# StanfordASL/GuSTO.jl

Measured on AMD Instinct MI355X. Metric: converged trajectories/sec (batched SCP), freeflyer_se2 N=50, inputs resident in HBM, higher is better.
Workload: dtype f64

## Files before the change

gusto.jl_amd/csrc/common.hpp:

```cpp
#pragma once
#include <hip/hip_runtime.h>
#include <math.h>
#include <stdint.h>

#include "gusto_hip.h"

namespace gusto {

#define GD __device__ __forceinline__
typedef double v4d __attribute__((ext_vector_type(4)));

constexpr int ROW_HARD = 0;
constexpr int ROW_PEN = 1;
constexpr int ROW_PEN_TR = 2;
constexpr int ROW_PEN_EQ = 3;
constexpr int ROW_HARD_EQ = 4;
constexpr int ROW_EQ = 5;
GD bool row_is_hard(int kind) { return kind == ROW_HARD || kind == ROW_HARD_EQ; }

constexpr int RS_T = 0, RS_LAM = 1, RS_LAMB = 2, RS_S = 3, RS_DT = 4, RS_DL = 5, RS_DS = 6, RS_KA = 7, RS_KB = 8,
              RS_NVAR = 9;

#ifndef GUSTO_DUBINS_WAVES
#define GUSTO_DUBINS_WAVES 2
#endif
#ifndef GUSTO_WAVES_PER_EU
#define GUSTO_WAVES_PER_EU 1
#endif

#ifndef GUSTO_TO_SWEEP_CALL
#define GUSTO_TO_SWEEP_CALL true
#endif
#ifndef GUSTO_TO4_SWEEP_CALL
#define GUSTO_TO4_SWEEP_CALL true
#endif
#ifndef GUSTO_USE_MFMA
#define GUSTO_USE_MFMA true
#endif
constexpr int GUSTO_TO_FREEFLYER_SE2 = 4, GUSTO_TO_ASTROBEE_SE3 = 5, GUSTO_TO_ASTROBEE_SE3_MANIFOLD = 6;
constexpr double TRAJOPT_DEFECT_REG = 1e-4;
constexpr int RS_EARLIER = 0, RS_ROW = 1, RS_ROW_LANE = 2;
template <int MODEL> struct MT;
template <> struct MT<GUSTO_FREEFLYER_SE2> {
    static constexpr int NDEF = 0;
    static constexpr int n = 6, m = 3, WS = 2, NFIX = 3, NHU = 2;
    static constexpr int WAVES_PER_EU = GUSTO_WAVES_PER_EU;
    static constexpr int RS_FORM = RS_ROW;
    static constexpr bool SWEEP_CALL = false;
    static constexpr bool MFMA = false;
    static constexpr int SCHED_PROBE = 2;
    static constexpr int SCHED_SLICE = 4;
    static constexpr bool LTI = true, HAS_OBS = true;
    static constexpr bool PG2 = true;
    static constexpr int pg_r0(int c) { return c < 3 ? c : (c < 6 ? c - 3 : c - 6); }
    static constexpr int pg_r1(int c) { return c < 3 ? c + 3 : (c < 6 ? c : c - 3); }
    static constexpr bool Anz(int i, int j) { return j == i + 3; }
    static constexpr bool Mnz(int i, int j) { return i == j || j == i + 3; }
    static constexpr bool Bnz(int i, int j) { return i == j + 3; }
    static constexpr bool Gnz(int i, int j) { return i == j || i == j + 3; }
    static constexpr bool Hnz(int, int) { return true; }
};
template <> struct MT<GUSTO_DUBINS_CAR> {
    static constexpr int NDEF = 0;
    static constexpr int n = 3, m = 1, WS = 2, NFIX = 6, NHU = 2;
    static constexpr int WAVES_PER_EU = GUSTO_DUBINS_WAVES;
    static constexpr int RS_FORM = RS_ROW;
    static constexpr bool SWEEP_CALL = false;
    static constexpr bool MFMA = false;
    static constexpr int SCHED_PROBE = 1; static constexpr int SCHED_SLICE = 0;
    static constexpr bool LTI = false, HAS_OBS = false;
    static constexpr bool PG2 = false;
    static constexpr int pg_r0(int) { return 0; }
    static constexpr int pg_r1(int) { return 0; }
    static constexpr bool Anz(int, int) { return true; }
    static constexpr bool Mnz(int, int) { return true; }
    static constexpr bool Bnz(int, int) { return true; }
    static constexpr bool Gnz(int, int) { return true; }
    static constexpr bool Hnz(int, int) { return true; }
};
template <> struct MT<GUSTO_ASTROBEE_SE3> {
    static constexpr int NDEF = 0;
    static constexpr int n = 12, m = 6, WS = 3, NFIX = 3, NHU = 2;
    static constexpr int WAVES_PER_EU = 1;
    static constexpr int RS_FORM = RS_ROW_LANE;
    static constexpr bool SWEEP_CALL = true;
    static constexpr bool MFMA = GUSTO_USE_MFMA;
    static constexpr int SCHED_PROBE = 1; static constexpr int SCHED_SLICE = 0;
    static constexpr bool LTI = false, HAS_OBS = true;
    static constexpr bool PG2 = false;
    static constexpr int pg_r0(int) { return 0; }
    static constexpr int pg_r1(int) { return 0; }
    static constexpr bool Anz(int i, int j) { return i < 3 ? j == i + 3 : (i < 6 ? false : (i < 9 ? j >= 6 : j >= 9)); }
    static constexpr bool Mnz(int i, int j) { return i < 3 ? (j == i || j == i + 3) : (i < 6 ? j == i : (i < 9 ? j >= 6 : j >= 9)); }
    static constexpr bool Bnz(int i, int j) { return j < 3 ? i == j + 3 : i == j + 6; }
    static constexpr bool Gnz(int i, int j) { return j < 3 ? (i == j || i == j + 3) : i >= 6; }
    static constexpr bool Hnz(int i, int j) { return i / 3 == j / 3; }
};
template <> struct MT<GUSTO_ASTROBEE_SE3_MANIFOLD> {
    static constexpr int NDEF = 0;
    static constexpr int n = 13, m = 6, WS = 3, NFIX = 5, NHU = 2;
    static constexpr int WAVES_PER_EU = 1;
    static constexpr int RS_FORM = RS_EARLIER;
    static constexpr bool SWEEP_CALL = true ;
    static constexpr bool MFMA = GUSTO_USE_MFMA;
    static constexpr int SCHED_PROBE = 1; static constexpr int SCHED_SLICE = 0;
    static constexpr bool LTI = false, HAS_OBS = true;
    static constexpr bool PG2 = false;
    static constexpr int pg_r0(int) { return 0; }
    static constexpr int pg_r1(int) { return 0; }
    static constexpr bool Anz(int i, int j) { return i < 3 ? j == i + 3 : (i < 6 ? false : (i < 10 ? j >= 6 : j >= 10)); }
    static constexpr bool Mnz(int i, int j) { return i < 3 ? (j == i || j == i + 3) : (i < 6 ? j == i : (i < 10 ? j >= 6 : j >= 10)); }
    static constexpr bool Bnz(int i, int j) { return j < 3 ? i == j + 3 : i == j + 7; }
    static constexpr bool Gnz(int i, int j) { return j < 3 ? (i == j || i == j + 3) : i >= 6; }
    static constexpr int hblk(int i) { return i < 3 ? 0 : (i < 6 ? 1 : (i < 10 ? 2 : 3)); }
    static constexpr bool Hnz(int i, int j) { return hblk(i) == hblk(j); }
};

template <> struct MT<GUSTO_TO_FREEFLYER_SE2> {
    using G = MT<GUSTO_FREEFLYER_SE2>;
    static constexpr int NDEF = 6, n = 6, m = 3 + NDEF, WS = 2, NFIX = 3, NHU = 2 + 2 * NDEF;
    static constexpr int WAVES_PER_EU = 1, SCHED_PROBE = 0, SCHED_SLICE = 0;
    static constexpr int RS_FORM = RS_ROW;
    static constexpr bool SWEEP_CALL = GUSTO_TO4_SWEEP_CALL, MFMA = false, LTI = false, HAS_OBS = true, PG2 = false;
    static constexpr int pg_r0(int) { return 0; }
    static constexpr int pg_r1(int) { return 0; }
    static constexpr bool Anz(int i, int j) { return G::Anz(i, j); }
    static constexpr bool Mnz(int i, int j) { return G::Mnz(i, j); }
    static constexpr bool Bnz(int i, int j) { return j < G::m && G::Bnz(i, j); }
    static constexpr bool Gnz(int i, int j) { return j < G::m ? G::Gnz(i, j) : i == j - G::m; }
    static constexpr bool Hnz(int, int) { return true; }
};
template <> struct MT<GUSTO_TO_ASTROBEE_SE3> {
    using G = MT<GUSTO_ASTROBEE_SE3>;
    static constexpr int NDEF = 12, n = 12, m = 6 + NDEF, WS = 3, NFIX = 3, NHU = 2 + 2 * NDEF;
    static constexpr int WAVES_PER_EU = 1, SCHED_PROBE = 0, SCHED_SLICE = 0;
    static constexpr int RS_FORM = RS_ROW;
    static constexpr bool SWEEP_CALL = GUSTO_TO_SWEEP_CALL, MFMA = false, LTI = false, HAS_OBS = true, PG2 = false;
    static constexpr int pg_r0(int) { return 0; }
    static constexpr int pg_r1(int) { return 0; }
    static constexpr bool Anz(int i, int j) { return G::Anz(i, j); }
    static constexpr bool Mnz(int i, int j) { return G::Mnz(i, j); }
    static constexpr bool Bnz(int i, int j) { return j < G::m && G::Bnz(i, j); }
    static constexpr bool Gnz(int i, int j) { return j < G::m ? G::Gnz(i, j) : i == j - G::m; }
    static constexpr bool Hnz(int, int) { return true; }
};

template <> struct MT<GUSTO_TO_ASTROBEE_SE3_MANIFOLD> {
    using G = MT<GUSTO_ASTROBEE_SE3_MANIFOLD>;
    static constexpr int NDEF = 13, n = 13, m = 6 + NDEF, WS = 3, NFIX = 5, NHU = 2 + 2 * NDEF;
    static constexpr int WAVES_PER_EU = 1, SCHED_PROBE = 0, SCHED_SLICE = 0;
    static constexpr int RS_FORM = RS_ROW;
    static constexpr bool SWEEP_CALL = GUSTO_TO_SWEEP_CALL, MFMA = false, LTI = false, HAS_OBS = true, PG2 = false;
    static constexpr int pg_r0(int) { return 0; }
    static constexpr int pg_r1(int) { return 0; }
    static constexpr bool Anz(int i, int j) { return G::Anz(i, j); }
    static constexpr bool Mnz(int i, int j) { return G::Mnz(i, j); }
    static constexpr bool Bnz(int i, int j) { return j < G::m && G::Bnz(i, j); }
    static constexpr bool Gnz(int i, int j) { return j < G::m ? G::Gnz(i, j) : i == j - G::m; }
    static constexpr bool Hnz(int, int) { return true; }
};
constexpr double TRAJOPT_EQ_DELTA = 1e-8;

inline void warm_defaults(int model, gusto_ipm_opts& io) {
    if (io.mu_floor < 0) io.mu_floor = (model == GUSTO_ASTROBEE_SE3_MANIFOLD) ? 1e-10 : 1e-11;
    if (io.sigma_max < 0) io.sigma_max = (model == GUSTO_TO_FREEFLYER_SE2 || model == GUSTO_TO_ASTROBEE_SE3 || model == GUSTO_TO_ASTROBEE_SE3_MANIFOLD) ? 0.0 : 0.1;
    if (!(io.mu_warm < 0)) { if (io.mu_warm_gain < 0) io.mu_warm_gain = 0.0; return; }
    switch (model) {
    case GUSTO_DUBINS_CAR: io.mu_warm = 1e-9; io.mu_warm_gain = 0.0; io.mu_warm_max = 1e-9; break;
    case GUSTO_FREEFLYER_SE2: io.mu_warm = 1e-4; io.mu_warm_gain = 0.1; io.mu_warm_max = 1e-2; break;
    case GUSTO_ASTROBEE_SE3: io.mu_warm = 1e-6; io.mu_warm_gain = 1.0; io.mu_warm_max = 1e-2; break;
    default: io.mu_warm = 1e-4; io.mu_warm_gain = 1.0; io.mu_warm_max = 1e-2; break;
    }
}
constexpr double IPM_DIVERGED = 1e3;
GD double warm_mu(const gusto_ipm_opts& io, double c) {
    if (io.mu_warm == 0.0) return 0.0;
    return fmin(fmax(io.mu_warm, io.mu_warm_max), fmax(io.mu_warm, io.mu_warm_gain * c * c));
}

GD constexpr int sidx(int i, int j, int n) {
    return i <= j ? i * n - i * (i - 1) / 2 + (j - i) : j * n - j * (j - 1) / 2 + (i - j);
}

template <int MODEL> struct Rec {
    using T = MT<MODEL>;
    static constexpr int n = T::n, m = T::m, NZ = n + m;
    static constexpr int r64(int c) { return (c + 63) / 64 * 64; }
    static constexpr bool S_TRI = false;
    static constexpr int NS = S_TRI ? m * (m + 1) / 2 : m * m;
    static constexpr int SQQ = r64(NZ * (NZ + 1) / 2), SNN = r64(n * n + 1), SKD = r64(2 * m * n + NS + 1);
    static constexpr int oK = 0, oD = m * n, oS = 2 * m * n;
    static constexpr int KD_DUMMY = 2 * m * n + NS;
    static constexpr int sS(int i, int l) {
        if (!S_TRI) return oS + i * m + l;
        const int a = i < l ? i : l, b = i < l ? l : i;
        return oS + a * m - a * (a - 1) / 2 + (b - a);
    }
};

template <int MODEL> struct SpPG {
    using T = MT<MODEL>;
    static constexpr int n = T::n, m = T::m;
    static constexpr int pos_phi(int l, int i) {
        int c = 0;
        for (int i2 = 0; i2 < n; i2++)
            for (int l2 = 0; l2 < n; l2++)
                if (T::Mnz(l2, i2) && (i2 < i || (i2 == i && l2 < l))) c++;
        return c;
    }
    static constexpr int NPHI = pos_phi(0, n);
    static constexpr int pos_gam(int l, int j) {
        int c = NPHI;
        for (int l2 = 0; l2 < n; l2++)
            for (int j2 = 0; j2 < m; j2++)
                if (T::Gnz(l2, j2) && (l2 < l || (l2 == l && j2 < j))) c++;
        return c;
    }
    static constexpr int NS = pos_gam(n, 0);
    static constexpr int S = (NS + 15) / 16 * 16;
    static constexpr bool USE = T::MFMA && T::NDEF == 0;
};

template <int MODEL> constexpr int rs_stride_rt(int N) { return MT<MODEL>::RS_FORM == RS_EARLIER ? N : (N + 63) & ~63; }
template <int MODEL, bool ONE> GD int rs_stride(int N) {
    if constexpr (ONE && MT<MODEL>::RS_FORM != RS_EARLIER) return 64;
    else return rs_stride_rt<MODEL>(N);
}
template <int MODEL, bool ONE> constexpr int rs_form() { return (ONE && MT<MODEL>::RS_FORM == RS_ROW_LANE) ? RS_ROW : MT<MODEL>::RS_FORM; }

struct WsLayout {
    int nslot;
    size_t rowstate, obs_nh, obs_c0, obs_mask, PG, PGS, QQ, Paft, Piaft, KD, Phicl, pvt, to_traj, total;
};
template <int MODEL> inline WsLayout make_ws_layout(int N, int n_obs) {
    using T = MT<MODEL>;
    constexpr int n = T::n, m = T::m, NZ = n + m;
    WsLayout L;
    L.nslot = T::NFIX + n_obs + 2 * n + T::NHU;
    size_t o = 0;
    auto take = [&](size_t c) { size_t r = o; o += (c + 1) & ~size_t(1); return r; };
    L.rowstate = take((size_t)RS_NVAR * L.nslot * rs_stride_rt<MODEL>(N));
    L.obs_nh = take((size_t)n_obs * T::WS * N);
    L.obs_c0 = take((size_t)n_obs * N);
    L.obs_mask = take((size_t)N);
    L.PG = take((size_t)(T::LTI ? 1 : N) * n * NZ);
    L.PGS = take(SpPG<MODEL>::USE ? (size_t)N * SpPG<MODEL>::S : 0);
    using R = Rec<MODEL>;
    L.QQ = take((size_t)N * R::SQQ);
    L.Paft = take((size_t)(N + 1) * R::SNN) + R::SNN;
    L.Piaft = take((size_t)(N + 1) * R::SNN) + R::SNN;
    L.KD = take((size_t)N * R::SKD);
    L.Phicl = take((size_t)N * R::SNN);
    L.pvt = take((size_t)N * (5 * n + 5 * m));
    L.to_traj = take(T::NDEF > 0 ? (size_t)2 * N * (n + m) : 0);
    L.total = T::RS_FORM == RS_EARLIER ? o : (o + 15) & ~size_t(15);
    return L;
}

template <int MODEL, bool ONE> struct LdsC {
    using T = MT<MODEL>;
    static constexpr int n = T::n, m = T::m, NZ = n + m;
    static constexpr bool BIG = n > 8;
    static constexpr int NPGB = (ONE && !T::LTI) ? 2 : 3;
    static constexpr int sP = 0, sPi = sP + n * n, sPG = sPi + n * n, sT0 = sPG + NPGB * n * NZ,
                         sHh = sT0 + ((ONE && BIG) ? 0 : n * NZ), sZ = sHh + NZ * NZ, sT = (ONE && BIG) ? sZ : sT0,
                         sGd = sZ + NZ * n, misc = sGd + ((ONE && BIG) ? 1 : 2) * n * n, sgoal = misc + 64 , lut = misc + 80,
                         vecs1w = (lut + (NZ * (NZ + 1) / 2 + 1) / 2 + 1 + 1) & ~1,
                         sK = vecs1w, sD = sK + m * n, sW = sD + m * n, sV = sW + m * n, vecsmw = sV + m * n,
                         vecs = ONE ? vecs1w : vecsmw;
    static constexpr int NVN = 7, NVM = 1;
    static constexpr bool KD_LDS = ONE && n <= 8;
    static constexpr bool PHI_FROM_K = KD_LDS && T::PG2;
    static constexpr bool PG_LDS = ONE && !T::LTI && n <= 4;
    static constexpr bool LC_LDS = ONE && MODEL == GUSTO_DUBINS_CAR;
    static constexpr int KDW = 2 * m * n + m * (m + 1) / 2;
    static constexpr int KDS = (KDW > NZ * (NZ + 1) / 2) ? KDW : NZ * (NZ + 1) / 2;
    static constexpr bool PHICL_LDS = n <= 8 && !PHI_FROM_K;
};
#ifndef GUSTO_SEG_W2
#ifdef GUSTO_STRICT_SYNC
#define GUSTO_SEG_W2 0
#else
#define GUSTO_SEG_W2 1
#endif
#endif
#ifndef GUSTO_SEG_MIN_N
#define GUSTO_SEG_MIN_N 4
#endif
template <int MODEL> constexpr bool seg2_big() { return GUSTO_SEG_W2 && MT<MODEL>::MFMA && MT<MODEL>::SWEEP_CALL && MT<MODEL>::NDEF == 0; }
__host__ __device__ constexpr int seg_lo(int c, int N, int NCH) { return (int)((long)N * c / NCH); }
constexpr int SEGW_FACTOR = 1, SEGW_BACK = 2, SEGW_FWD = 3, SEGW_ROWS_R = 5, SEGW_STEP = 6, SEGW_STEP_CS = 7, SEGW_EXIT = 9;
constexpr int SEG_RP = 15;
template <int MODEL, int NCH> struct SegB {
    static constexpr int n = MT<MODEL>::n, m = MT<MODEL>::m, NNp = (n * n + 1) & ~1, NPG = n * (n + m), NI = NCH - 1;
    static constexpr int IFB = 7 * NNp, Tt = 0, Sg = NNp, Pa = 2 * NNp, A2 = 3 * NNp, A3 = 4 * NNp, Pc = 5 * NNp, PIc = 6 * NNp;
    static constexpr int IF(int j) { return j * IFB; }
    static constexpr int CHB = 3 * NNp, Pf = 0, Pif = NNp, Gdf = 2 * NNp;
    static constexpr int CH(int c) { return NI * IFB + c * CHB; }
    static constexpr int COM = NI * (IFB + CHB), Gci = COM, A1 = COM + NNp, X1 = COM + 2 * NNp, X2 = COM + 3 * NNp;
    static constexpr int vec = COM + 4 * NNp;
    static constexpr int XI(int j) { return vec + 16 * j; }
    static constexpr int LAM(int j) { return vec + 16 * NI + 16 * j; }
    static constexpr int PBV(int c) { return vec + 32 * NI + 16 * (c - 1); }
    static constexpr int hlp = vec + 48 * NI, HLB = (2 * NPG + 64 > SEG_RP * 64) ? 2 * NPG + 64 : SEG_RP * 64;
// ... 373 lines not shown
```

gusto.jl_amd/csrc/ipm.hpp:

```cpp
#pragma once
#include "rows.hpp"

#ifndef GUSTO_COOP_CHOL_MIN
#define GUSTO_COOP_CHOL_MIN 7
#endif

namespace gusto {

extern __shared__ __attribute__((aligned(16))) double gusto_dyn_lds[];

template <int MODEL> constexpr bool costate_adjoint();

struct IpmOut {
    int status, iters;
    double obj, res_p, res_d, mu;
};

template <bool ONEWAVE> GD void blk_sync() {
    if constexpr (ONEWAVE) {
#ifdef GUSTO_STRICT_SYNC
        asm volatile("s_waitcnt vmcnt(0) lgkmcnt(0)\n\ts_barrier" ::: "memory");
#endif
        __builtin_amdgcn_fence(__ATOMIC_ACQ_REL, "wavefront");
        __builtin_amdgcn_wave_barrier();
// ... 1088 lines not shown
                    for (int l = 0; l < n; l++) pb[l] = ex[sg * n + l];
#pragma unroll
                    for (int l = 0; l < n; l++) acc[l % PS] += col[l] * pb[l];
                } else {
                    double pb[n];
#pragma unroll
                    for (int l = 0; l < n; l++) pb[l] = readlane_f64(pval, sg * n + l);
                    __builtin_amdgcn_sched_barrier(0);
#pragma unroll
                    for (int l = 0; l < n; l++) acc[l % PS] += col[l] * pb[l];
                }
                const double s = (PS == 4) ? (acc[0] + acc[1]) + (acc[2] + acc[PS - 1]) : acc[0];
                pval = (g == gs) ? s : pval;
                if constexpr (XL) ex[tid] = pval;
            }
        }
        {
            const int kk = k0 - g;
            if (tid < C * n && kk >= 1) K.pv[(kk - 1) * n + i] = pval;
        }
#pragma unroll
        for (int l = 0; l < n; l++) col[l] = coln[l];
        qv = qvn;
    }
    K.sync();
}

template <class BLKA> GD void forward_sweep_1w(BLKA K) {
    using BLK = std::remove_cv_t<std::remove_reference_t<BLKA>>;
    constexpr int n = BLK::n, C = 64 / n, PS = n > 8 ? 4 : 1;
    constexpr bool XL = n > 8;
    double* ex = K.sHh;
    using R = typename BLK::R;
    const int tid = K.tid, N = K.N;
    const int g = (tid < C * n) ? tid / n : C - 1, i = (tid < C * n) ? tid % n : 0;
    double gi = 0.0;
    auto phi_e = [&](int r_, int c_) { return (r_ == c_) ? 1.0 : ((c_ == r_ + n / 2) ? K.dt : 0.0); };
    if constexpr (BLK::C::PHI_FROM_K) {
        constexpr int m = BLK::m;
        double Bd[n * m];
        Dyn<BLK::MODEL_ID>::B(*K.mpp, Bd);
        const double h = 0.5 * K.dt;
#pragma unroll
        for (int l = 0; l < n; l++) {
            const int c_ = l % m;
            const double hb = h * Bd[(c_ + n / 2) * m + c_];
            const double gv = (l < n / 2) ? 2.0 * (h * hb) : 2.0 * hb;
            gi = (i == l) ? gv : gi;
        }
    }
    double phr[n];
#pragma unroll
    for (int l = 0; l < n; l++) phr[l] = phi_e(i, l);
    double row[n], rown[n], cv, cvn = 0, yval = 0.0;
    auto fetch = [&](int k0, double* r, double& c) {
        const int kk = (k0 + g < N) ? k0 + g : N - 1;
        if constexpr (BLK::C::PHI_FROM_K) {
            constexpr int m = BLK::m;
            const int ic = (i < m) ? i : i - m;
#pragma unroll
            for (int l = 0; l < n; l++) r[l] = phr[l] - gi * K.kdl[kk * BLK::C::KDS + ic * n + l];
        } else if constexpr (n <= 4) {
            const bool ok = k0 + g < N;
#pragma unroll
            for (int l = 0; l < n; l++) r[l] = ok ? K.Phicl[(size_t)kk * BLK::SPH + i * n + l] : 0.0;
            c = ok ? K.dY[kk * n + i] : 0.0;
            return;
        } else {
#pragma unroll
            for (int l = 0; l < n; l++) r[l] = K.Phicl[(size_t)kk * BLK::SPH + i * n + l];
        }
        c = K.dY[kk * n + i];
    };
    constexpr int RING = (XL && !BLK::C::KD_LDS) ? GUSTO_SWEEP_RING : 1;
    if constexpr (RING > 1) {
        double rb[RING][n], qb[RING];
#pragma unroll
        for (int d = 0; d < RING - 1; d++) fetch(d * C, rb[d], qb[d]);
        ex[tid] = yval;
        K.sync();
        for (int kb = 0; kb < N; kb += RING * C) {
            static_for<0, RING>([&](auto DD) {
                constexpr int d = decltype(DD)::value;
                const int k0 = kb + d * C;
                fetch(k0 + (RING - 1) * C, rb[(d + RING - 1) % RING], qb[(d + RING - 1) % RING]);
                if (k0 < N) {
#pragma unroll
                    for (int gs = 0; gs < C; gs++) {
                        if (k0 + gs < N) {
                            const int sg = (gs == 0) ? C - 1 : gs - 1;
                            double acc[PS];
#pragma unroll
                            for (int q = 0; q < PS; q++) acc[q] = (q == 0) ? qb[d] : 0.0;
                            double pb[n];
#pragma unroll
                            for (int l = 0; l < n; l++) pb[l] = readlane_f64(yval, sg * n + l);
                            __builtin_amdgcn_sched_barrier(0);
#pragma unroll
                            for (int l = 0; l < n; l++) acc[l % PS] += rb[d][l] * pb[l];
                            const double s = (PS == 4) ? (acc[0] + acc[1]) + (acc[2] + acc[PS - 1]) : acc[0];
                            yval = (g == gs) ? s : yval;
                        }
                    }
                    const int kk = k0 + g;
                    if (tid < C * n && kk < N) K.dY[kk * n + i] = yval;
                }
            });
        }
        K.sync();
        return;
    }
    fetch(0, row, cv);
    if constexpr (XL) ex[tid] = yval;
    K.sync();
    for (int k0 = 0; k0 < N; k0 += C) {
        if (k0 + C < N) fetch(k0 + C, rown, cvn);
#pragma unroll
        for (int gs = 0; gs < C; gs++) {
            if (k0 + gs < N) {
                const int sg = (gs == 0) ? C - 1 : gs - 1;
                double acc[PS];
#pragma unroll
                for (int q = 0; q < PS; q++) acc[q] = (q == 0) ? cv : 0.0;
                if constexpr (XL) {
                    double pb[n];
#pragma unroll
                    for (int l = 0; l < n; l++) pb[l] = ex[sg * n + l];
#pragma unroll
                    for (int l = 0; l < n; l++) acc[l % PS] += row[l] * pb[l];
                } else {
                    double pb[n];
#pragma unroll
                    for (int l = 0; l < n; l++) pb[l] = readlane_f64(yval, sg * n + l);
                    __builtin_amdgcn_sched_barrier(0);
#pragma unroll
                    for (int l = 0; l < n; l++) acc[l % PS] += row[l] * pb[l];
                }
                const double s = (PS == 4) ? (acc[0] + acc[1]) + (acc[2] + acc[PS - 1]) : acc[0];
                yval = (g == gs) ? s : yval;
                if constexpr (XL) ex[tid] = yval;
            }
        }
        {
            const int kk = k0 + g;
            if (tid < C * n && kk < N) K.dY[kk * n + i] = yval;
        }
#pragma unroll
        for (int l = 0; l < n; l++) row[l] = rown[l];
        cv = cvn;
    }
    K.sync();
}

template <int MODEL> GD void costate_pass_1w(SweepView<MODEL> K, const double* mugn) {
    using T = MT<MODEL>;
    using R = Rec<MODEL>;
    constexpr int n = T::n, C = 64 / n;
    const int tid = K.tid, N = K.N;
    const int g = (tid < C * n) ? tid / n : C - 1, i = (tid < C * n) ? tid % n : 0;
    double mg[n];
#pragma unroll
    for (int l = 0; l < n; l++) mg[l] = mugn[l];
    constexpr int RING = GUSTO_SWEEP_RING;
    double pr[RING][n], pi[RING][n];
    auto fetch = [&](int k0, double* a, double* b) {
        const int k = (k0 + g + 1 < N) ? k0 + g : N - 2;
        const double* pa = K.Paft + (size_t)k * R::SNN + (T::MFMA ? i : i * n);
        const double* pb = K.Piaft + (size_t)k * R::SNN + (T::MFMA ? i : i * n);
#pragma unroll
        for (int l = 0; l < n; l++) { a[l] = pa[T::MFMA ? l * n : l]; b[l] = pb[T::MFMA ? l * n : l]; }
    };
#pragma unroll
    for (int d = 0; d < RING - 1; d++) fetch(d * C, pr[d], pi[d]);
    for (int kb = 0; kb + 1 < N; kb += RING * C) {
        static_for<0, RING>([&](auto DD) {
            constexpr int d = decltype(DD)::value;
            const int k0 = kb + d * C;
            fetch(k0 + (RING - 1) * C, pr[(d + RING - 1) % RING], pi[(d + RING - 1) % RING]);
            if (k0 + 1 < N) {
                const bool ok = tid < C * n && k0 + g + 1 < N;
                const int k = (k0 + g + 1 < N) ? k0 + g : N - 2;
                double s = K.pv[k * n + i] - K.rv[k * n + i];
#pragma unroll
                for (int l = 0; l < n; l++) s += pr[d][l] * K.dY[k * n + l] + pi[d][l] * mg[l];
                if (ok) K.nun[(k + 1) * n + i] = s;
            }
        });
    }
    K.sync();
}
template <int MODEL> __device__ __noinline__ void costate_pass_1w_call(typename Blk<MODEL, true>::Args a) {
    Blk<MODEL, true> B(a, gusto_dyn_lds);
    costate_pass_1w<MODEL>(SweepView<MODEL>::make(B), gusto_dyn_lds + LdsC<MODEL, true>::misc + 48);
}


template <int MODEL> constexpr bool adjoint_pattern_ok() {
    using T = MT<MODEL>;
    constexpr int n = T::n, q = n - 9;
    for (int i = 0; i < n; i++)
        for (int l = 0; l < n; l++) {
            const bool want = (i < 6) ? (l == i || (i >= 3 && l == i - 3)) : (l >= 6 && l < ((i < 6 + q) ? 6 + q : n));
            if (want != T::Mnz(l, i)) return false;
        }
    return true;
}
template <int MODEL> GD void adjoint_sweep_1w(SweepView<MODEL> K) {
    using T = MT<MODEL>;
    constexpr int n = T::n, NZ = T::n + T::m, C = 64 / n, q = n - 9, NR = n - 6;
    static_assert(adjoint_pattern_ok<MODEL>(), "column pattern of M of the astrobee models");
    const int tid = K.tid, N = K.N;
    const int g = (tid < C * n) ? tid / n : C - 1, i = (tid < C * n) ? tid % n : 0;
    int rl[NR];
    bool rok[NR];
    const int hi = (i < 6 + q) ? 6 + q : n;
#pragma unroll
    for (int j = 0; j < NR; j++) {
        rl[j] = (i < 6) ? ((j == 1 && i >= 3) ? i - 3 : i) : 6 + j;
        rok[j] = (i < 6) ? (j == 0 || (j == 1 && i >= 3)) : (6 + j < hi);
        if (!rok[j]) rl[j] = i;
    }
    int cs = 0, pj[NR];
#pragma unroll
    for (int i2 = 0; i2 < n; i2++) cs = (i == i2) ? SpPG<MODEL>::pos_phi(0, i2) : cs;
#pragma unroll
    for (int j = 0; j < NR; j++) pj[j] = (i < 6) ? ((i >= 3) ? (j == 1 ? 0 : (j == 0 ? 1 : 0)) : 0) : (rok[j] ? j : 0);
    double* ex = K.sHh;
    constexpr int RING = GUSTO_SWEEP_RING;
    double cb[RING][NR], vb[RING];
    auto fetch = [&](int k0, double* c, double& v) {
        const int kk = (k0 - g >= 1) ? k0 - g : 1;
        const auto pg = K.PGS + (size_t)kk * SpPG<MODEL>::S + cs;
#pragma unroll
        for (int j = 0; j < NR; j++) { const double a = pg[pj[j]]; c[j] = rok[j] ? a : 0.0; }
        v = K.nun[kk * n + i];
    };
#pragma unroll
    for (int d = 0; d < RING - 1; d++) fetch(N - 2 - d * C, cb[d], vb[d]);
    double val = K.nun[(N - 1) * n + i];
    ex[tid] = val;
    K.sync();
    for (int kb = N - 2; kb >= 1; kb -= RING * C) {
        static_for<0, RING>([&](auto DD) {
            constexpr int d = decltype(DD)::value;
            const int k0 = kb - d * C;
            fetch(k0 - (RING - 1) * C, cb[(d + RING - 1) % RING], vb[(d + RING - 1) % RING]);
            if (k0 >= 1) {
#pragma unroll
                for (int gs = 0; gs < C; gs++) {
                    if (k0 - gs >= 1) {
                        const int sg = (gs == 0) ? C - 1 : gs - 1;
                        double pb[NR];
#pragma unroll
                        for (int j = 0; j < NR; j++) pb[j] = ex[sg * n + rl[j]];
                        double s = vb[d];
#pragma unroll
                        for (int j = 0; j < NR; j++) s += cb[d][j] * pb[j];
                        val = (g == gs) ? s : val;
                        ex[tid] = val;
                    }
                }
                const int kk = k0 - g;
                if (tid < C * n && kk >= 1) K.nun[kk * n + i] = val;
            }
        });
    }
    K.sync();
}
template <int MODEL> __device__ __noinline__ void adjoint_sweep_1w_call(typename Blk<MODEL, true>::Args a, double hdt) {
    using T = MT<MODEL>;
    constexpr int n = T::n, m = T::m;
    Blk<MODEL, true> K(a, gusto_dyn_lds);
    adjoint_sweep_1w<MODEL>(SweepView<MODEL>::make(K));
    if (K.tid == 0) {
        const double* gxs = gusto_dyn_lds + LdsC<MODEL, true>::misc + 16;
        double Ad[n * n], x0[n], u0[m];
#pragma unroll
        for (int i = 0; i < n; i++) x0[i] = K.Xp[i];
#pragma unroll
        for (int i = 0; i < m; i++) u0[i] = K.Up[i];
        Dyn<MODEL>::A(K.P.mp, x0, u0, Ad);
#pragma unroll
        for (int i = 0; i < n; i++) {
            double s = gxs[i] + K.nun[n + i];
#pragma unroll
            for (int j = 0; j < n; j++) if (T::Anz(j, i)) s += hdt * Ad[j * n + i] * K.nun[n + j];
            K.nun[i] = -s;
        }
    }
    K.sync();
}

template <int MODEL> __device__ __noinline__ void factor_sweep_1w_call(typename Blk<MODEL, true>::Args a, Prof* pf) {
    Blk<MODEL, true> B(a, gusto_dyn_lds);
    SweepView<MODEL> K = SweepView<MODEL>::make(B);
    if constexpr (MT<MODEL>::MFMA) {
        if constexpr (!costate_adjoint<MODEL>()) factor_sweep_mfma<MODEL, false>(K, gusto_dyn_lds + LdsC<MODEL, true>::misc + 8, *pf);
        else if (costate_adjoint_now<MODEL>()) factor_sweep_mfma<MODEL, true>(K, gusto_dyn_lds + LdsC<MODEL, true>::misc + 8, *pf);
        else factor_sweep_mfma<MODEL, false>(K, gusto_dyn_lds + LdsC<MODEL, true>::misc + 8, *pf);
    }
    else factor_sweep_1w<MODEL>(K, gusto_dyn_lds + LdsC<MODEL, true>::misc + 8, *pf);
}
template <int MODEL, class BLK> __device__ __noinline__ void factor_sweep_mw_call(typename BLK::Args a, Prof* pf) {
    BLK K(a, gusto_dyn_lds);
    if constexpr (MT<MODEL>::m >= GUSTO_COOP_CHOL_MIN) {
        if (K.NTr <= 64) { factor_sweep_w1<MODEL>(K, gusto_dyn_lds + BLK::C::misc + 8, *pf); return; }
    }
    factor_sweep_mw<MODEL>(K, gusto_dyn_lds + BLK::C::misc + 8, *pf);
}
template <class BLK> __device__ __noinline__ void backward_sweep_mw_call(typename BLK::Args a) {
    BLK K(a, gusto_dyn_lds);
    if (K.NTr <= 64) backward_sweep_1w<const BLK&>(K); else backward_sweep_mw(K);
}
template <class BLK> __device__ __noinline__ void forward_sweep_mw_call(typename BLK::Args a) {
    BLK K(a, gusto_dyn_lds);
    if (K.NTr <= 64) forward_sweep_1w<const BLK&>(K); else forward_sweep_mw(K);
}
template <int MODEL, class BLK> GD void factor_sweep(BLK& K, double* fail, Prof& pf) {
    if constexpr (!BLK::ONE && MT<MODEL>::SWEEP_CALL && MT<MODEL>::NDEF > 0) factor_sweep_mw_call<MODEL, BLK>(K.args(), &pf);
    else if constexpr (!BLK::ONE) factor_sweep_mw<MODEL>(K, fail, pf);
    else if constexpr (MT<MODEL>::SWEEP_CALL) factor_sweep_1w_call<MODEL>(K.args(), &pf);
    else if constexpr (MT<MODEL>::MFMA) factor_sweep_mfma<MODEL, false>(SweepView<MODEL>::make(K), fail, pf);
    else if constexpr (MT<MODEL>::PG2 && LdsC<MODEL, true>::KD_LDS) {
        factor_sweep_pg2<MODEL>(SweepView<MODEL>::make(K), fail, pf);
    }
    else factor_sweep_1w<MODEL>(SweepView<MODEL>::make(K), fail, pf);
}
template <int MODEL> __device__ __noinline__ void backward_sweep_1w_call(typename Blk<MODEL, true>::Args a) {
    Blk<MODEL, true> B(a, gusto_dyn_lds);
    backward_sweep_1w(SweepView<MODEL>::make(B));
}
template <int MODEL> __device__ __noinline__ void forward_sweep_1w_call(typename Blk<MODEL, true>::Args a) {
    Blk<MODEL, true> B(a, gusto_dyn_lds);
    forward_sweep_1w(SweepView<MODEL>::make(B));
}
template <int MODEL, class BLK> GD void backward_sweep(BLK& K) {
    if constexpr (!BLK::ONE && MT<MODEL>::SWEEP_CALL && MT<MODEL>::NDEF > 0) backward_sweep_mw_call<BLK>(K.args());
    else if constexpr (!BLK::ONE) backward_sweep_mw(K);
    else if constexpr (MT<MODEL>::SWEEP_CALL) backward_sweep_1w_call<MODEL>(K.args());
    else backward_sweep_1w(SweepView<MODEL>::make(K));
}
template <int MODEL, class BLK> GD void forward_sweep(BLK& K) {
    if constexpr (!BLK::ONE && MT<MODEL>::SWEEP_CALL && MT<MODEL>::NDEF > 0) forward_sweep_mw_call<BLK>(K.args());
    else if constexpr (!BLK::ONE) forward_sweep_mw(K);
    else if constexpr (MT<MODEL>::SWEEP_CALL) forward_sweep_1w_call<MODEL>(K.args());
    else forward_sweep_1w(SweepView<MODEL>::make(K));
}

template <int MODEL, class BLK> GD void inv_spd_block(BLK& K, double* fail) {
    constexpr int n = BLK::n;
    const int tid = K.tid, nt = K.nt();
    double* A = K.sGd;
    double* Li = K.sHh;
    if constexpr (BLK::ONE) {
        const int r = tid < n ? tid : n - 1;
        double a[n];
#pragma unroll
        for (int c = 0; c < n; c++) { a[c] = A[r * n + c]; if (c == r && !K.is_goal(r)) a[c] = 1.0; }
        bool bad = false;
        static_for<0, n>([&](auto J) {
            constexpr int j = decltype(J)::value;
            const double ajj = readlane_f64(a[j], j);
            if (!(ajj > 0.0)) bad = true;
            const double d = rsqrt_nr(ajj);
            a[j] = (r >= j) ? a[j] * d : a[j];
            static_for<j + 1, n>([&](auto C) {
                constexpr int c = decltype(C)::value;
                const double lcj = readlane_f64(a[j], c);
                double t = a[c];
                t -= a[j] * lcj;
                a[c] = (r >= c) ? t : a[c];
            });
        });
        if (bad) *fail = 1.0;
        double x[n];
        static_for<0, n>([&](auto I) {
            constexpr int i = decltype(I)::value;
            const double ri = rcp_nr(readlane_f64(a[i], i));
            double acc = 0;
            static_for<0, i>([&](auto L_) {
                constexpr int l = decltype(L_)::value;
                acc -= readlane_f64(a[l], i) * x[l];
            });
            x[i] = (i == r) ? ri : ((i > r) ? acc * ri : 0.0);
        });
        if (tid < n) {
#pragma unroll
            for (int i = 0; i < n; i++) Li[i * n + tid] = x[i];
        }
        K.sync();
#pragma unroll
        for (int t = 0; t < (n * n + 63) / 64; t++) {
            const int e = tid + 64 * t, ec = e < n * n ? e : n * n - 1;
            const int i = ec / n, j = ec % n;
            double acc = 0;
#pragma unroll
            for (int l = 0; l < n; l++) acc += Li[l * n + i] * Li[l * n + j];
            if (e < n * n) K.sP[e] = acc;
        }
        return;
    }
    for (int e = tid; e < n * n; e += nt) {
        const int i = e / n, j = e % n;
        if (i == j && !K.is_goal(i)) A[e] = 1.0;
        Li[e] = 0.0;
    }
    K.sync();
    for (int j = 0; j < n; j++) {
        const double ajj = A[j * n + j];
        if (!(ajj > 0.0)) *fail = 1.0;
        const double d = rsqrt_nr(ajj);
        K.sync();
        if (tid >= j && tid < n) A[tid * n + j] *= d;
        K.sync();
        for (int e = tid; e < n * n; e += nt) {
            const int i = e / n, c = e % n;
            if (c > j && i >= c) A[e] -= A[i * n + j] * A[c * n + j];
        }
        K.sync();
    }
    if (tid < n) {
        const int c = tid;
        Li[c * n + c] = rcp_nr(A[c * n + c]);
        for (int i = c + 1; i < n; i++) {
            double acc = 0;
            for (int l = c; l < i; l++) acc -= A[i * n + l] * Li[l * n + c];
            Li[i * n + c] = acc * rcp_nr(A[i * n + i]);
        }
    }
    K.sync();
    for (int e = tid; e < n * n; e += nt) {
        const int i = e / n, j = e % n;
        double acc = 0;
        for (int l = (i > j ? i : j); l < n; l++) acc += Li[l * n + i] * Li[l * n + j];
        K.sP[e] = acc;
    }
}

template <int MODEL, class BLK, int NCH = 0> GD void mid_phase(BLK& K, int k, bool act, double hdt, double* red, double* mugn, Prof* pf = nullptr) {
    constexpr bool SEG = NCH > 0;
#define MT_(i) do { if (pf) pf->tick(i); } while (0)
    MT_(PF_MID);
    using T = MT<MODEL>;
    using R = Rec<MODEL>;
    constexpr int n = T::n, m = T::m, NZ = n + m;
    const int N = K.N;
    double th[n], d0[m];
    constexpr bool KEEP_D = T::SWEEP_CALL && BLK::ONE && !BLK::C::KD_LDS;
    double Dk[KEEP_D ? m * n : 1];
#pragma unroll
    for (int i = 0; i < (KEEP_D ? m * n : 1); i++) Dk[i] = 0;
#pragma unroll
    for (int i = 0; i < n; i++) th[i] = 0;
#pragma unroll
    for (int i = 0; i < m; i++) d0[i] = 0;
    if (act) {
        double tt[n], lu[m], Gamk[n * m];
        constexpr bool GT_RECOMP = !T::LTI && n > 8 && T::NDEF == 0;
        double gterm[n], gsub[n];
        if (k >= 1) {
            if constexpr (T::PG2 || (!T::LTI && n > 8 && T::NDEF == 0)) {
                double Mk_[n * n];
                load_M_Gam(K, k, Mk_, Gamk);
                if constexpr (GT_RECOMP) {
#pragma unroll
                    for (int j = 0; j < n; j++) {
                        double g = 0.0;
#pragma unroll
                        for (int i = 0; i < n; i++) if (T::Mnz(j, i)) g += Mk_[j * n + i] * K.rd_(k, i);
                        gterm[j] = g; gsub[j] = K.misc[64 + j] - K.Xw[k * n + j];
                    }
                }
            } else {
                const auto pg = K.PGk(k);
#pragma unroll
                for (int i = 0; i < n; i++)
#pragma unroll
                    for (int j = 0; j < m; j++) Gamk[i * m + j] = T::Gnz(i, j) ? pg[i * NZ + n + j] : 0.0;
            }
        } else {
            Dyn<MODEL>::B(K.P.mp, Gamk);
#pragma unroll
            for (int i = 0; i < n * m; i++) Gamk[i] *= hdt;
            if constexpr (T::NDEF > 0) {
#pragma unroll
                for (int i = 0; i < T::NDEF; i++) Gamk[i * m + (m - T::NDEF) + i] = 1.0;
            }
        }
#pragma unroll
        for (int i = 0; i < n; i++) tt[i] = K.pv[k * n + i];
#pragma unroll
        for (int i = 0; i < m; i++) {
            double s = K.qu_(k, i);
#pragma unroll
            for (int l = 0; l < n; l++) if (T::Gnz(l, i)) s += Gamk[l * m + i] * tt[l];
            lu[i] = s;
        }
#pragma unroll
// ... 1032 lines not shown
```

Before: 138,700.

## Add DPP-based backward/forward sweep for freeflyer SE2 single-wave path

Adds new backward and forward Riccati-style sweep kernels for the freeflyer SE2 model. They propagate the 6-vector recurrence across lanes using v_fmac_f64_dpp row_newbcast broadcasts and permlane16/32 swaps, so each step's matrix-vector product and its hand-off to the next time step stay in registers instead of passing through LDS or readlane. Eight time steps are mapped onto two 6-lane groups per 16-lane row, with loads prefetched one chunk ahead. The new path is enabled by default for this model only. It relies on inline assembly with a hand-placed s_nop hazard pad and on gfx950-specific permlane swap builtins.

```diff
diff --git a/gusto.jl_amd/csrc/common.hpp b/gusto.jl_amd/csrc/common.hpp
--- a/gusto.jl_amd/csrc/common.hpp
+++ b/gusto.jl_amd/csrc/common.hpp
@@ -33,6 +33,9 @@
 #endif
 #ifndef GUSTO_TO4_SWEEP_CALL
 #define GUSTO_TO4_SWEEP_CALL true
+#endif
+#ifndef GUSTO_SWEEP_DPP
+#define GUSTO_SWEEP_DPP 1
 #endif
 #ifndef GUSTO_USE_MFMA
 #define GUSTO_USE_MFMA true
@@ -47,6 +50,7 @@
     static constexpr int WAVES_PER_EU = GUSTO_WAVES_PER_EU;
     static constexpr int RS_FORM = RS_ROW;
     static constexpr bool SWEEP_CALL = false;
+    static constexpr bool SWEEP_DPP = GUSTO_SWEEP_DPP;
     static constexpr bool MFMA = false;
     static constexpr int SCHED_PROBE = 2;
     static constexpr int SCHED_SLICE = 4;
@@ -66,6 +70,7 @@
     static constexpr int WAVES_PER_EU = GUSTO_DUBINS_WAVES;
     static constexpr int RS_FORM = RS_ROW;
     static constexpr bool SWEEP_CALL = false;
+    static constexpr bool SWEEP_DPP = false;
     static constexpr bool MFMA = false;
     static constexpr int SCHED_PROBE = 1; static constexpr int SCHED_SLICE = 0;
     static constexpr bool LTI = false, HAS_OBS = false;
@@ -84,6 +89,7 @@
     static constexpr int WAVES_PER_EU = 1;
     static constexpr int RS_FORM = RS_ROW_LANE;
     static constexpr bool SWEEP_CALL = true;
+    static constexpr bool SWEEP_DPP = false;
     static constexpr bool MFMA = GUSTO_USE_MFMA;
     static constexpr int SCHED_PROBE = 1; static constexpr int SCHED_SLICE = 0;
     static constexpr bool LTI = false, HAS_OBS = true;
@@ -102,6 +108,7 @@
     static constexpr int WAVES_PER_EU = 1;
     static constexpr int RS_FORM = RS_EARLIER;
     static constexpr bool SWEEP_CALL = true ;
+    static constexpr bool SWEEP_DPP = false;
     static constexpr bool MFMA = GUSTO_USE_MFMA;
     static constexpr int SCHED_PROBE = 1; static constexpr int SCHED_SLICE = 0;
     static constexpr bool LTI = false, HAS_OBS = true;
@@ -121,6 +128,7 @@
     static constexpr int NDEF = 6, n = 6, m = 3 + NDEF, WS = 2, NFIX = 3, NHU = 2 + 2 * NDEF;
     static constexpr int WAVES_PER_EU = 1, SCHED_PROBE = 0, SCHED_SLICE = 0;
     static constexpr int RS_FORM = RS_ROW;
+    static constexpr bool SWEEP_DPP = false;
     static constexpr bool SWEEP_CALL = GUSTO_TO4_SWEEP_CALL, MFMA = false, LTI = false, HAS_OBS = true, PG2 = false;
     static constexpr int pg_r0(int) { return 0; }
     static constexpr int pg_r1(int) { return 0; }
@@ -135,6 +143,7 @@
     static constexpr int NDEF = 12, n = 12, m = 6 + NDEF, WS = 3, NFIX = 3, NHU = 2 + 2 * NDEF;
     static constexpr int WAVES_PER_EU = 1, SCHED_PROBE = 0, SCHED_SLICE = 0;
     static constexpr int RS_FORM = RS_ROW;
+    static constexpr bool SWEEP_DPP = false;
     static constexpr bool SWEEP_CALL = GUSTO_TO_SWEEP_CALL, MFMA = false, LTI = false, HAS_OBS = true, PG2 = false;
     static constexpr int pg_r0(int) { return 0; }
     static constexpr int pg_r1(int) { return 0; }
@@ -150,6 +159,7 @@
     static constexpr int NDEF = 13, n = 13, m = 6 + NDEF, WS = 3, NFIX = 5, NHU = 2 + 2 * NDEF;
     static constexpr int WAVES_PER_EU = 1, SCHED_PROBE = 0, SCHED_SLICE = 0;
     static constexpr int RS_FORM = RS_ROW;
+    static constexpr bool SWEEP_DPP = false;
     static constexpr bool SWEEP_CALL = GUSTO_TO_SWEEP_CALL, MFMA = false, LTI = false, HAS_OBS = true, PG2 = false;
     static constexpr int pg_r0(int) { return 0; }
     static constexpr int pg_r1(int) { return 0; }
diff --git a/gusto.jl_amd/csrc/ipm.hpp b/gusto.jl_amd/csrc/ipm.hpp
--- a/gusto.jl_amd/csrc/ipm.hpp
+++ b/gusto.jl_amd/csrc/ipm.hpp
@@ -1264,6 +1264,149 @@
     K.sync();
 }
 
+template <int HOP> GD double row_hop(double x, double g) {
+    const unsigned long long ux = __builtin_bit_cast(unsigned long long, x), ug = __builtin_bit_cast(unsigned long long, g);
+    const unsigned xl = (unsigned)ux, xh = (unsigned)(ux >> 32), gl = (unsigned)ug, gh = (unsigned)(ug >> 32);
+    unsigned lo, hi;
+    if constexpr (HOP == 0) { lo = __builtin_amdgcn_permlane16_swap(gl, xl, false, false)[0]; hi = __builtin_amdgcn_permlane16_swap(gh, xh, false, false)[0]; }
+    if constexpr (HOP == 1) { lo = __builtin_amdgcn_permlane32_swap(gl, xl, false, false)[0]; hi = __builtin_amdgcn_permlane32_swap(gh, xh, false, false)[0]; }
+    if constexpr (HOP == 2) { lo = __builtin_amdgcn_permlane16_swap(xl, gl, false, false)[1]; hi = __builtin_amdgcn_permlane16_swap(xh, gh, false, false)[1]; }
+    if constexpr (HOP == 3) { lo = __builtin_amdgcn_permlane32_swap(xl, gl, false, false)[1]; hi = __builtin_amdgcn_permlane32_swap(xh, gh, false, false)[1]; }
+    return __builtin_bit_cast(double, ((unsigned long long)hi << 32) | lo);
+}
+template <int HALF> GD double dpp_step6(double p, double q, const double* c) {
+    double acc = q;
+    if constexpr (HALF == 0)
+        asm("s_nop 1\n\tv_fmac_f64_dpp %0, %1, %2 row_newbcast:0 row_mask:0xf bank_mask:0xf\n\tv_fmac_f64_dpp %0, %1, %3 row_newbcast:1 row_mask:0xf bank_mask:0xf\n\t"
+            "v_fmac_f64_dpp %0, %1, %4 row_newbcast:2 row_mask:0xf bank_mask:0xf\n\tv_fmac_f64_dpp %0, %1, %5 row_newbcast:3 row_mask:0xf bank_mask:0xf\n\t"
+            "v_fmac_f64_dpp %0, %1, %6 row_newbcast:4 row_mask:0xf bank_mask:0xf\n\tv_fmac_f64_dpp %0, %1, %7 row_newbcast:5 row_mask:0xf bank_mask:0xf"
+            : "+v"(acc) : "v"(p), "v"(c[0]), "v"(c[1]), "v"(c[2]), "v"(c[3]), "v"(c[4]), "v"(c[5]));
+    else
+        asm("s_nop 1\n\tv_fmac_f64_dpp %0, %1, %2 row_newbcast:8 row_mask:0xf bank_mask:0xf\n\tv_fmac_f64_dpp %0, %1, %3 row_newbcast:9 row_mask:0xf bank_mask:0xf\n\t"
+            "v_fmac_f64_dpp %0, %1, %4 row_newbcast:10 row_mask:0xf bank_mask:0xf\n\tv_fmac_f64_dpp %0, %1, %5 row_newbcast:11 row_mask:0xf bank_mask:0xf\n\t"
+            "v_fmac_f64_dpp %0, %1, %6 row_newbcast:12 row_mask:0xf bank_mask:0xf\n\tv_fmac_f64_dpp %0, %1, %7 row_newbcast:13 row_mask:0xf bank_mask:0xf"
+            : "+v"(acc) : "v"(p), "v"(c[0]), "v"(c[1]), "v"(c[2]), "v"(c[3]), "v"(c[4]), "v"(c[5]));
+    return acc;
+}
+template <class LIVE> GD void dpp_chunk(double& p, double& keep, double q, const double* c, int g, LIVE live) {
+    static_for<0, 8>([&](auto GS) {
+        constexpr int gs = decltype(GS)::value;
+        if (live(gs)) {
+            const double acc = dpp_step6<(gs & 1) ? 0 : 1>(p, q, c);
+            keep = (g == gs) ? acc : keep;
+            if constexpr (gs & 1) p = row_hop<gs / 2>(acc, p); else p = acc;
+        }
+    });
+}
+template <class BLKA> GD void backward_sweep_dpp(BLKA K) {
+    using BLK = std::remove_cv_t<std::remove_reference_t<BLKA>>;
+    constexpr int n = BLK::n, m = BLK::m, C = 8;
+    static_assert(n == 6 && BLK::C::PHI_FROM_K, "two groups of 6 lanes per row, operands from K");
+    const int tid = K.tid, N = K.N;
+    const int row = tid >> 4, j = tid & 15;
+    const bool act = (j & 7) < n;
+    const int g = 2 * (row ^ (row >> 1)) + (j >> 3), i = act ? (j & 7) : 0;
+    double gl[n];
+    auto phi_e = [&](int r_, int c_) { return (r_ == c_) ? 1.0 : ((c_ == r_ + n / 2) ? K.dt : 0.0); };
+    {
+        double Bd[n * m];
+        Dyn<BLK::MODEL_ID>::B(*K.mpp, Bd);
+        const double h = 0.5 * K.dt;
+#pragma unroll
+        for (int l = 0; l < n; l++) {
+            const int c_ = l % m;
+            const double hb = h * Bd[(c_ + n / 2) * m + c_];
+            gl[l] = (l < n / 2) ? 2.0 * (h * hb) : 2.0 * hb;
+        }
+    }
+    double phc[n];
+#pragma unroll
+    for (int l = 0; l < n; l++) phc[l] = phi_e(l, i);
+    double col[n], kc[m], qv, qvn, p, keep = 0.0;
+    auto load = [&](int k0, double& q) {
+        const int kk = (k0 - g >= 1) ? k0 - g : 1;
+#pragma unroll
+        for (int a = 0; a < m; a++) kc[a] = K.kdl[kk * BLK::C::KDS + a * n + i];
+        q = K.pv[kk * n + i];
+    };
+    auto form = [&]() {
+#pragma unroll
+        for (int l = 0; l < n; l++) col[l] = phc[l] - gl[l] * kc[l % m];
+    };
+    load(N - 1, qv);
+    form();
+    p = K.rv[(N - 1) * n + i];
+    K.sync();
+    if (tid < n) K.pv[(N - 1) * n + tid] = p;
+    for (int k0 = N - 1; k0 >= 1; k0 -= C) {
+        load(k0 - C, qvn);
+        if (k0 - (C - 1) >= 1) dpp_chunk(p, keep, qv, col, g, [](int) { return true; });
+        else dpp_chunk(p, keep, qv, col, g, [&](int gs) { return k0 - gs >= 1; });
+        {
+            const int kk = k0 - g;
+            if (act && kk >= 1) K.pv[(kk - 1) * n + i] = keep;
+        }
+        __builtin_amdgcn_sched_barrier(0);
+        form();
+        qv = qvn;
+    }
+    K.sync();
+}
+template <class BLKA> GD void forward_sweep_dpp(BLKA K) {
+    using BLK = std::remove_cv_t<std::remove_reference_t<BLKA>>;
+    constexpr int n = BLK::n, m = BLK::m, C = 8;
+    static_assert(n == 6 && BLK::C::PHI_FROM_K, "two groups of 6 lanes per row, operands from K");
+    const int tid = K.tid, N = K.N;
+    const int row = tid >> 4, j = tid & 15;
+    const bool act = (j & 7) < n;
+    const int g = 2 * (row ^ (row >> 1)) + (j >> 3), i = act ? (j & 7) : 0;
+    double gi = 0.0;
+    auto phi_e = [&](int r_, int c_) { return (r_ == c_) ? 1.0 : ((c_ == r_ + n / 2) ? K.dt : 0.0); };
+    {
+        double Bd[n * m];
+        Dyn<BLK::MODEL_ID>::B(*K.mpp, Bd);
+        const double h = 0.5 * K.dt;
+#pragma unroll
+        for (int l = 0; l < n; l++) {
+            const int c_ = l % m;
+            const double hb = h * Bd[(c_ + n / 2) * m + c_];
+            const double gv = (l < n / 2) ? 2.0 * (h * hb) : 2.0 * hb;
+            gi = (i == l) ? gv : gi;
+        }
+    }
+    double phr[n];
+#pragma unroll
+    for (int l = 0; l < n; l++) phr[l] = phi_e(i, l);
+    double rw[n], kr[n], cv, cvn, p = 0.0, keep = 0.0;
+    auto load = [&](int k0, double& c) {
+        const int kk = (k0 + g < N) ? k0 + g : N - 1;
+        const int ic = (i < m) ? i : i - m;
+#pragma unroll
+        for (int l = 0; l < n; l++) kr[l] = K.kdl[kk * BLK::C::KDS + ic * n + l];
+        c = K.dY[kk * n + i];
+    };
+    auto form = [&]() {
+#pragma unroll
+        for (int l = 0; l < n; l++) rw[l] = phr[l] - gi * kr[l];
+    };
+    load(0, cv);
+    form();
+    K.sync();
+    for (int k0 = 0; k0 < N; k0 += C) {
+        load(k0 + C, cvn);
+        if (k0 + C - 1 < N) dpp_chunk(p, keep, cv, rw, g, [](int) { return true; });
+        else dpp_chunk(p, keep, cv, rw, g, [&](int gs) { return k0 + gs < N; });
+        {
+            const int kk = k0 + g;
+            if (act && kk < N) K.dY[kk * n + i] = keep;
+        }
+        __builtin_amdgcn_sched_barrier(0);
+        form();
+        cv = cvn;
+    }
+    K.sync();
+}
+
 template <int MODEL> GD void costate_pass_1w(SweepView<MODEL> K, const double* mugn) {
     using T = MT<MODEL>;
     using R = Rec<MODEL>;
@@ -1450,12 +1593,14 @@
     if constexpr (!BLK::ONE && MT<MODEL>::SWEEP_CALL && MT<MODEL>::NDEF > 0) backward_sweep_mw_call<BLK>(K.args());
     else if constexpr (!BLK::ONE) backward_sweep_mw(K);
     else if constexpr (MT<MODEL>::SWEEP_CALL) backward_sweep_1w_call<MODEL>(K.args());
+    else if constexpr (MT<MODEL>::SWEEP_DPP) backward_sweep_dpp(SweepView<MODEL>::make(K));
     else backward_sweep_1w(SweepView<MODEL>::make(K));
 }
 template <int MODEL, class BLK> GD void forward_sweep(BLK& K) {
     if constexpr (!BLK::ONE && MT<MODEL>::SWEEP_CALL && MT<MODEL>::NDEF > 0) forward_sweep_mw_call<BLK>(K.args());
     else if constexpr (!BLK::ONE) forward_sweep_mw(K);
     else if constexpr (MT<MODEL>::SWEEP_CALL) forward_sweep_1w_call<MODEL>(K.args());
+    else if constexpr (MT<MODEL>::SWEEP_DPP) forward_sweep_dpp(SweepView<MODEL>::make(K));
     else forward_sweep_1w(SweepView<MODEL>::make(K));
 }
 
```

After: 143,400, median of 6. +3.4%, better.
